# bruAristimunha/Synthetic-Sleep-EEG-Signal-Generation-using-Latent-Diffusion-Models

Hardware: AMD Instinct MI355X
Metric: EEG windows/sec (LDM train step) (higher is better)
Workload: dtype bf16; 1 GPU; LDM train step on raw (B,1,3072) windows: frozen AutoencoderKL[32,32,64] encode+sample x scale, add_noise, config_ldm.yaml UNet (30.5M params, latent_channels=1) fwd+bwd, epsilon MSE, Adam lr 1e-4 [BASELINE configs[2]/[3]: per-GPU batch 256 = global 2048 / 8]; per_gpu_batch=256, global_batch=256, latent_len=768, parallelism=dp1

## Files before the change

include/eegldm.h:

```cpp
#ifndef EEGLDM_H
#define EEGLDM_H
#include <stdint.h>
#ifdef __cplusplus
extern "C" {
#endif

#define EEGLDM_ABI_VERSION 8

enum { EEGLDM_F32 = 0, EEGLDM_BF16 = 1, EEGLDM_F16 = 2 };
enum {
  EEGLDM_OK = 0,
  EEGLDM_ERR_INVALID = -1,
  EEGLDM_ERR_HIP = -2,
  EEGLDM_ERR_UNSUPPORTED = -3,
  EEGLDM_ERR_NOMEM = -4
};
enum { EEGLDM_PRED_EPSILON = 0, EEGLDM_PRED_V = 1, EEGLDM_PRED_SAMPLE = 2 };

typedef struct eegldm_ctx eegldm_ctx;
typedef struct eegldm_unet eegldm_unet;
typedef struct eegldm_aekl eegldm_aekl;
typedef struct eegldm_disc eegldm_disc;
typedef struct eegldm_block eegldm_block;

int eegldm_abi_version(void);
const char* eegldm_last_error(void);
int eegldm_ctx_create(int hip_device, void* hip_stream, int own_stream, eegldm_ctx** out);
void* eegldm_ctx_stream(const eegldm_ctx*);
int eegldm_ctx_destroy(eegldm_ctx* ctx);
int eegldm_ctx_sync(eegldm_ctx* ctx);
int eegldm_timer_start(eegldm_ctx* ctx);
int eegldm_timer_stop_ms(eegldm_ctx* ctx, float* ms_host);
int eegldm_prof_enable(eegldm_ctx* ctx, int on);
int eegldm_prof_summary(eegldm_ctx* ctx, int kernel_class, double* flops_host, double* ms_host, int* launches_host);
int eegldm_prof_bracket_overhead_ms(eegldm_ctx* ctx, double* ms_host);
int eegldm_prof_dump(eegldm_ctx* ctx, const char* path_host);
int eegldm_debug_reload_env(void);
int eegldm_debug_gn_last_route(int backward, int* out6_host);

int eegldm_ncl_to_nlc(eegldm_ctx*, const float* src_ncl, void* dst_nlc, long ld_dst, int B, int C, int L, int dst_dtype);
int eegldm_nlc_to_ncl(eegldm_ctx*, const void* src_nlc, long ld_src, float* dst_ncl, int B, int C, int L, int src_dtype);
int eegldm_pack_conv_weight(eegldm_ctx*, const float* w_ref, float* w_packed, int Cout, int Cin, int K);
int eegldm_unpack_conv_weight(eegldm_ctx*, const float* w_packed, float* w_ref, int Cout, int Cin, int K);
int eegldm_cast(eegldm_ctx*, const float* src, void* dst, long n, int dst_dtype);

int eegldm_conv1d_pack_kblocked(eegldm_ctx*, const void* w, void* w_kblocked, int Cout, int Cin, int dtype);
int eegldm_conv1d_pack_kblocked_k(eegldm_ctx*, const void* w, void* w_kblocked, int Cout, int Cin, int K, int dtype);
int eegldm_conv1d_forget_kblocked(eegldm_ctx*, const void* w);
int eegldm_conv1d_pack_stride2(eegldm_ctx*, const void* w, void* w_fwd, void* w_dgrad, int Cout, int Cin, int dtype);
int eegldm_conv1d_pack_dgrad(eegldm_ctx*, const void* w, void* w_dgrad, int Cout, int Cin, int dtype);
int eegldm_conv1d_pack_dgrad_k(eegldm_ctx*, const void* w, void* w_dgrad, int Cout, int Cin, int K, int dtype);

int eegldm_conv1d_fwd(eegldm_ctx*, const void* x, long ldx, const void* w, const float* bias,
                      void* y, long ldy, int B, int Lin, int Cin, int Cout, int K, int stride,
                      int pad_l, int pad_r, const float* rowvec, long ld_rowvec,
                      const void* resid, long ld_resid, int dtype);
int eegldm_conv1d_skip_fwd(eegldm_ctx*, const void* x, long ldx, const void* w, const float* bias,
                           const void* x2, long ldx2, const void* w2, const float* bias2, void* y, long ldy,
                           int B, int L, int Cin, int Cin2, int Cout, const float* rowvec, long ld_rowvec, int dtype);
int eegldm_conv1d_bwd_data(eegldm_ctx*, const void* dy, long lddy, const void* w, void* dx, long lddx,
                           int B, int Lin, int Cin, int Cout, int K, int stride, int pad_l, int pad_r,
                           const void* resid, long ld_resid, int dtype);
int eegldm_conv1d_bwd_weight(eegldm_ctx*, const void* x, long ldx, const void* dy, long lddy,
                             float* dw, float* dbias, int B, int Lin, int Cin, int Cout, int K,
                             int stride, int pad_l, int pad_r, int dtype);
int eegldm_linear_fwd(eegldm_ctx*, const void* x, long ldx, const void* w, const float* bias, void* y, long ldy,
                      int M, int N, int K, int dtype, int out_f32);
int eegldm_linear_bwd(eegldm_ctx*, const void* x, long ldx, const void* w, const void* dy, long lddy, void* dx, long lddx,
                      float* dw, float* dbias, int M, int N, int K, int dtype, int dx_f32);

int eegldm_groupnorm_fwd(eegldm_ctx*, const void* x, long ldx, const float* gamma, const float* beta,
// ... 274 lines not shown
```

synthetic-sleep-eeg-signal-generation-using-latent-diffusion-models_amd/_lib.py:

```python
import ctypes as C
import os

_HERE = os.path.dirname(os.path.abspath(__file__))
LIB_PATH = os.environ.get("EEGLDM_LIB") or os.path.join(_HERE, "libeegldm.so")

F32, BF16, F16 = 0, 1, 2
PRED = {"epsilon": 0, "v_prediction": 1, "sample": 2}


class LibraryMissing(RuntimeError):
    pass


def _load():
    import torch
    if not os.path.exists(LIB_PATH):
        raise LibraryMissing(f"{LIB_PATH} not found: build it with `make` (python -c 'import __graft_entry__ as g; g.build()')")
    return C.CDLL(LIB_PATH)


lib = _load()
lib.eegldm_last_error.restype = C.c_char_p
if hasattr(lib, "eegldm_ctx_stream"):
    lib.eegldm_ctx_stream.restype = C.c_void_p
if hasattr(lib, 'eegldm_unet_num_params'):
    lib.eegldm_unet_num_params.restype = C.c_long

_vp, _i, _l, _f = C.c_void_p, C.c_int, C.c_long, C.c_float
SIGNATURES = {
    "eegldm_abi_version": [],
    "eegldm_last_error": [],
    "eegldm_ctx_create": [_i, _vp, _i, C.POINTER(_vp)],
    "eegldm_ctx_stream": [_vp],
    "eegldm_ctx_destroy": [_vp],
    "eegldm_ctx_sync": [_vp],
    "eegldm_timer_start": [_vp],
    "eegldm_timer_stop_ms": [_vp, C.POINTER(_f)],
    "eegldm_prof_enable": [_vp, _i],
    "eegldm_prof_summary": [_vp, _i, C.POINTER(C.c_double), C.POINTER(C.c_double), C.POINTER(_i)],
    "eegldm_prof_bracket_overhead_ms": [_vp, C.POINTER(C.c_double)],
    "eegldm_prof_dump": [_vp, C.c_char_p],
    "eegldm_debug_reload_env": [],
    "eegldm_debug_gn_last_route": [_i, _vp],
    "eegldm_ncl_to_nlc": [_vp, _vp, _vp, _l, _i, _i, _i, _i],
    "eegldm_nlc_to_ncl": [_vp, _vp, _l, _vp, _i, _i, _i, _i],
    "eegldm_pack_conv_weight": [_vp, _vp, _vp, _i, _i, _i],
    "eegldm_conv1d_pack_kblocked": [_vp, _vp, _vp, _i, _i, _i],
    "eegldm_conv1d_pack_kblocked_k": [_vp, _vp, _vp, _i, _i, _i, _i],
    "eegldm_batchnorm_lrelu_fwd": [_vp, _vp, _l, _vp, _vp, _vp, _vp, _vp, _vp, _vp, _l, _l, _i, _f, _i, _i],
    "eegldm_batchnorm_lrelu_bwd": [_vp, _vp, _l, _vp, _vp, _vp, _vp, _l, _vp, _l, _vp, _vp, _l, _i, _f, _i],
    "eegldm_kl_reparam_fwd": [_vp, _vp, _vp, _vp, _vp, _vp, _vp, _l, _i, _i],
    "eegldm_kl_reparam_bwd": [_vp, _vp, _vp, _vp, _vp, _vp, _vp, _vp, _l, _f, _i],
    "eegldm_avgpool2_fwd": [_vp, _vp, _l, _vp, _l, _i, _i, _i, _i],
    "eegldm_avgpool2_bwd": [_vp, _vp, _l, _vp, _l, _i, _i, _i, _i],
    "eegldm_nearest2_fwd": [_vp, _vp, _l, _vp, _l, _i, _i, _i, _i],
    "eegldm_nearest2_bwd": [_vp, _vp, _l, _vp, _l, _i, _i, _i, _i],
    "eegldm_conv1d_skip_fwd": [_vp, _vp, _l, _vp, _vp, _vp, _l, _vp, _vp, _vp, _l, _i, _i, _i, _i, _i, _vp, _l, _i],
    "eegldm_comm_unique_id": [_vp],
    "eegldm_comm_create": [_vp, _vp, _i, _i, _vp],
    "eegldm_comm_destroy": [_vp],
    "eegldm_comm_rank": [_vp],
    "eegldm_comm_world": [_vp],
    "eegldm_comm_allreduce_mean_f32": [_vp, _vp, _l, _l],
    "eegldm_comm_broadcast_f32": [_vp, _vp, _l, _i],
    "eegldm_comm_wait": [_vp],
    "eegldm_conv1d_forget_kblocked": [_vp, _vp],
    "eegldm_conv1d_pack_stride2": [_vp, _vp, _vp, _vp, _i, _i, _i],
    "eegldm_conv1d_pack_dgrad": [_vp, _vp, _vp, _i, _i, _i],
    "eegldm_conv1d_pack_dgrad_k": [_vp, _vp, _vp, _i, _i, _i, _i],
    "eegldm_unpack_conv_weight": [_vp, _vp, _vp, _i, _i, _i],
    "eegldm_cast": [_vp, _vp, _vp, _l, _i],
    "eegldm_conv1d_fwd": [_vp, _vp, _l, _vp, _vp, _vp, _l, _i, _i, _i, _i, _i, _i, _i, _i, _vp, _l, _vp, _l, _i],
    "eegldm_conv1d_bwd_data": [_vp, _vp, _l, _vp, _vp, _l, _i, _i, _i, _i, _i, _i, _i, _i, _vp, _l, _i],
    "eegldm_conv1d_bwd_weight": [_vp, _vp, _l, _vp, _l, _vp, _vp, _i, _i, _i, _i, _i, _i, _i, _i, _i],
    "eegldm_linear_fwd": [_vp, _vp, _l, _vp, _vp, _vp, _l, _i, _i, _i, _i, _i],
    "eegldm_linear_bwd": [_vp, _vp, _l, _vp, _vp, _l, _vp, _l, _vp, _vp, _i, _i, _i, _i, _i],
# ... 244 lines not shown
```

synthetic-sleep-eeg-signal-generation-using-latent-diffusion-models_amd/csrc/aekl.hip:

```cpp
#include <stdlib.h>

#include <string>
#include <vector>

#include "aekl_thin.h"
#include "net.h"

int ls_bn_lrelu_fwd(eegldm_ctx*, const void* x, long ldx, const float* gamma, const float* beta, float* stats, float* rmean, float* rvar,
                    float* nbt, void* y, long ldy, long rows, int C, float slope, int training, int dtype);
int ls_bn_lrelu_bwd(eegldm_ctx*, const void* x, long ldx, const float* gamma, const float* beta, const float* stats, const void* dy, long lddy,
                    void* dx, long lddx, float* dgamma, float* dbeta, long rows, int C, float slope, int dtype);
int ls_bn_stats(eegldm_ctx*, const void* x, long ldx, float* stats, float* rmean, float* rvar, float* nbt, long rows, int C, int training, int dtype);
int ls_bn_stats_from_parts(eegldm_ctx*, const float* parts, int nb, float* stats, float* rmean, float* rvar, float* nbt, long rows, int C);
int ls_bn_apply(eegldm_ctx*, const void* x, long ldx, const float* gamma, const float* beta, const float* stats, void* y, long ldy, long rows, int C, float slope, int dtype);
bool disc_tail_ok(int dtype, int C, long ldy);
int disc_tail_fwd(eegldm_ctx*, int dtype, const void* y, long ldy, const float* gamma, const float* beta, const float* stats, const float* w3,
                  const float* bias, float slope, float* logits, int B, int L, int C);
int disc_tail_bwd(eegldm_ctx*, int dtype, const void* y, long ldy, const float* gamma, const float* beta, const float* stats, const float* w3,
                  float slope, const float* dlogits, void* dy, long lddy, float* dgamma, float* dbeta, float* dw3, float* dbias, int B, int L, int C);
bool disc_head_ok(int dtype, int C0, long ldda, int stride, int L, int Lo);
int disc_head_bwd(eegldm_ctx*, int dtype, const void* da, long ldda, const void* x, const void* w, const float* bias, float slope,
                  float* dw, float* db, float* dx, int B, int L, int Lo, int C0, int stride);
int ls_upsample2(eegldm_ctx*, const void* x, long ldx, void* y, long ldy, long rows_in, int C, int dtype);
int ls_upsample2_bwd(eegldm_ctx*, const void* dy, long lddy, void* dx, long lddx, long rows_in, int C, int dtype);
// ... 360 lines not shown
    int ic = oc; oc = nc[i];
    for (int r = 0; r < cfg->num_res_blocks; r++) { dec.push_back(make_res(a, lay, dname(""), ic, oc, G)); bi++; ic = oc; }
    if (i != 0) {
      Op u; u.kind = OP_UPS; dec.push_back(u);
      dec.push_back(make_conv(a, lay, dname(".conv.conv"), ic, ic, 3, 1, 1, 1, true)); bi++;
    }
  }
  dec.push_back(make_gn(a, lay, dname(""), oc, G)); bi++;
  dec.push_back(make_conv(a, lay, dname(".conv"), oc, cfg->out_channels, 3, 1, 1, 1, true)); bi++;
  a->q_mu = make_conv(a, lay, "quant_conv_mu.conv", lat, lat, 1, 1, 0, 0, true);
  a->q_lv = make_conv(a, lay, "quant_conv_log_sigma.conv", lat, lat, 1, 1, 0, 0, true);
  a->dec.push_back(make_conv(a, lay, "post_quant_conv.conv", lat, lat, 1, 1, 0, 0, true));
  for (auto& o : dec) a->dec.push_back(o);
  a->nparams = lay.off;
  *out = a;
  return 0;
}
eegldm_ctx* aekl_ctx(const eegldm_aekl* a) { return a->ctx; }
int aekl_out_channels(const eegldm_aekl* a) { return a->cfg.out_channels; }
int aekl_down(const eegldm_aekl* a) { return 1 << (a->cfg.n_levels - 1); }
extern "C" int eegldm_aekl_destroy(eegldm_aekl* a) { delete a; return 0; }
extern "C" int eegldm_aekl_num_entries(const eegldm_aekl* a) { return (int)a->entries.size(); }
extern "C" long eegldm_aekl_num_params(const eegldm_aekl* a) { return a->nparams; }
extern "C" int eegldm_aekl_entry(const eegldm_aekl* a, int i, char* name, int cap, long* offset, long* numel, int* ndim, int shape[3]) {
  return entry_query(a, i, name, cap, offset, numel, ndim, shape);
}
extern "C" int eegldm_aekl_bind(eegldm_aekl* a, float* params, float* grads) { EEG_CHECK(a && params, "null argument"); return a->bind(params, grads); }
extern "C" int eegldm_aekl_sync_weights(eegldm_aekl* a) { EEG_CHECK(a, "null argument"); return a->sync_weights(); }

namespace {
int lat_len(const eegldm_aekl* a, int L) { return L >> (a->cfg.n_levels - 1); }

bool enc_fused_eligible(const eegldm_aekl* a, int L);
int aekl_encode_fused_seq(eegldm_aekl* a, View x, int B, int& L, View* out);
int aekl_encode_impl(eegldm_aekl* a, const float* x, const float* eps, int B, int L, View* z_out, float* kl, bool frozen = false) {
  EEG_CHECK((L % (1 << (a->cfg.n_levels - 1))) == 0, "L=%d must be divisible by 2^(levels-1)", L);
  eegldm_ctx* ctx = a->ctx; const int dt = a->dtype, lat = a->cfg.latent_channels, cin = a->cfg.in_channels;
  a->arena.reset(); a->rt.clear(); a->tape_enc.clear(); a->tape_dec.clear();
  a->B = B; a->L = L; a->have_tape = false;
  View x0; ALLOC_OR_FAIL(x0.p, a->alloc_act((long)B * L, cin)); x0.ld = cin; x0.C = cin;
  EEG_TRY(eegldm_ncl_to_nlc(ctx, x, x0.p, cin, B, cin, L, dt));
  int Lc = L;
  if (frozen && enc_fused_eligible(a, L)) EEG_TRY(aekl_encode_fused_seq(a, x0, B, Lc, &a->h_enc));
  else EEG_TRY(a->forward_seq(a->enc, x0, B, Lc, &a->h_enc, a->tape_enc, 1));
  a->Ll = Lc;
  const long n = (long)B * Lc * lat;
  ALLOC_OR_FAIL(a->mu.p, a->alloc_act((long)B * Lc, lat)); a->mu.ld = lat; a->mu.C = lat;
  ALLOC_OR_FAIL(a->lv.p, a->alloc_act((long)B * Lc, lat)); a->lv.ld = lat; a->lv.C = lat;
  EEG_TRY(op_conv_fwd(ctx, dt, a->h_enc.p, a->h_enc.ld, a->W(a->q_mu.w), a->P(a->q_mu.b), a->mu.p, lat, B, Lc, lat, lat, 1, 1, 0, 0, nullptr, 0, nullptr, 0));
  EEG_TRY(op_conv_fwd(ctx, dt, a->h_enc.p, a->h_enc.ld, a->W(a->q_lv.w), a->P(a->q_lv.b), a->lv.p, lat, B, Lc, lat, lat, 1, 1, 0, 0, nullptr, 0, nullptr, 0));
  a->eps_nlc = nullptr;
  if (eps) {
    ALLOC_OR_FAIL(a->eps_nlc, a->arena.alloc(sizeof(float) * n));
    EEG_TRY(eegldm_ncl_to_nlc(ctx, eps, a->eps_nlc, lat, B, lat, Lc, EEGLDM_F32));
  }
  ALLOC_OR_FAIL(a->sigma, a->arena.alloc(sizeof(float) * n));
  View z; ALLOC_OR_FAIL(z.p, a->alloc_act((long)B * Lc, lat)); z.ld = lat; z.C = lat;
  if (kl && !ctx->loss_prezeroed) HIP_TRY(hipMemsetAsync(kl, 0, sizeof(float), ctx->stream));
  EEG_TRY(ls_reparam(ctx, a->mu.p, a->lv.p, a->eps_nlc, z.p, a->sigma, kl, n, B, dt));
  *z_out = z;
  return 0;
}
bool enc_fused_eligible(const eegldm_aekl* a, int L) {
  if (getenv("EEGLDM_AEKL_NO_FUSED_ENC") != nullptr) return false;
  if ((a->dtype != EEGLDM_BF16 && a->dtype != EEGLDM_F16) || a->cfg.norm_num_groups != 1) return false;
  int Lc = L; bool any = false;
  for (const Op& o : a->enc) {
    if (o.kind == OP_CONV) Lc = (Lc + o.pl + o.pr - o.k) / o.stride + 1;
    else if (o.kind == OP_RES) { if (!pre_conv3_ok(a->dtype, o.r.cin, o.r.cout, Lc) || !pre_conv3_ok(a->dtype, o.r.cout, o.r.cout, Lc)) return false; any = true; }
    else if (o.kind != OP_GN) return false;
  }
  return any;
}
int aekl_encode_fused_seq(eegldm_aekl* a, View x, int B, int& L, View* out) {
  eegldm_ctx* ctx = a->ctx; const int dt = a->dtype;
  size_t nslots = 0;
  for (const Op& o : a->enc) nslots += (o.kind == OP_RES) ? 2 : 0;
  double* slots; ALLOC_OR_FAIL(slots, (double*)a->arena.alloc(sizeof(double) * 2 * B * (nslots + 1)));
  HIP_TRY(hipMemsetAsync(slots, 0, sizeof(double) * 2 * B * (nslots + 1), ctx->stream));
  size_t used = 0;
  auto next_slot = [&]() { return slots + (used++) * 2 * (size_t)B; };
  double* cur_stats = nullptr;
  for (size_t i = 0; i < a->enc.size(); i++) {
    const Op& o = a->enc[i];
    const bool next_res = i + 1 < a->enc.size() && a->enc[i + 1].kind == OP_RES;
    if (o.kind == OP_CONV) {
      const int Lo = (L + o.pl + o.pr - o.k) / o.stride + 1;
      View y; ALLOC_OR_FAIL(y.p, a->alloc_act((long)B * Lo, o.cout)); y.ld = o.cout; y.C = o.cout;
      EEG_TRY(op_conv_fwd(ctx, dt, x.p, x.ld, a->W(o.w), o.b >= 0 ? a->P(o.b) : nullptr, y.p, y.ld, B, L, o.cin, o.cout, o.k, o.stride, o.pl, o.pr,
                          nullptr, 0, nullptr, 0));
      L = Lo; x = y; cur_stats = nullptr;
      if (next_res) { cur_stats = next_slot(); EEG_TRY(sample_stats_launch(ctx, x.p, (long)L * x.C, B, cur_stats, a->dtype)); }
    } else if (o.kind == OP_RES) {
      const ResDesc& r = o.r;
      EEG_CHECK(cur_stats, "fused encoder: no statistics for a ResBlock input");
      View h1; ALLOC_OR_FAIL(h1.p, a->alloc_act((long)B * L, r.cout)); h1.ld = r.cout; h1.C = r.cout;
      double* st_h1 = next_slot();
      EEG_TRY(pre_conv3_launch(ctx, x.p, cur_stats, a->P(r.gn1_w), a->P(r.gn1_b), a->W(r.c1_w), a->P(r.c1_b), nullptr, h1.p, st_h1, B, L, r.cin, r.cout, GN_EPS, a->dtype));
      View res = x;
      if (r.sk_w >= 0) {
        ALLOC_OR_FAIL(res.p, a->alloc_act((long)B * L, r.cout)); res.ld = r.cout; res.C = r.cout;
        EEG_TRY(op_conv_fwd(ctx, dt, x.p, x.ld, a->W(r.sk_w), a->P(r.sk_b), res.p, res.ld, B, L, r.cin, r.cout, 1, 1, 0, 0, nullptr, 0, nullptr, 0));
      }
      View y; ALLOC_OR_FAIL(y.p, a->alloc_act((long)B * L, r.cout)); y.ld = r.cout; y.C = r.cout;
      double* st_y = next_res ? next_slot() : nullptr;
      EEG_TRY(pre_conv3_launch(ctx, h1.p, st_h1, a->P(r.gn2_w), a->P(r.gn2_b), a->W(r.c2_w), a->P(r.c2_b), res.p, y.p, st_y, B, L, r.cout, r.cout, GN_EPS, a->dtype));
      x = y; cur_stats = st_y;
    } else {
      View y; ALLOC_OR_FAIL(y.p, a->alloc_act((long)B * L, x.C)); y.ld = x.C; y.C = x.C;
      float* st; ALLOC_OR_FAIL(st, (float*)a->arena.alloc(sizeof(float) * 2 * B * o.groups));
      EEG_TRY(eegldm_groupnorm_fwd(ctx, x.p, x.ld, a->P(o.gw), a->P(o.gb), y.p, y.ld, st, B, L, x.C, o.groups, GN_EPS, 0, 0, nullptr, 0, dt));
      x = y; cur_stats = nullptr;
    }
  }
  *out = x;
  return 0;
}

int aekl_export_latents(eegldm_aekl* a, const View& z, float* z_ncl, float* mu_ncl, float* sigma_ncl) {
  const int lat = a->cfg.latent_channels;
  if (z_ncl) EEG_TRY(eegldm_nlc_to_ncl(a->ctx, z.p, lat, z_ncl, a->B, lat, a->Ll, a->dtype));
  if (mu_ncl) EEG_TRY(eegldm_nlc_to_ncl(a->ctx, a->mu.p, lat, mu_ncl, a->B, lat, a->Ll, a->dtype));
  if (sigma_ncl) EEG_TRY(eegldm_nlc_to_ncl(a->ctx, a->sigma, lat, sigma_ncl, a->B, lat, a->Ll, EEGLDM_F32));
  return 0;
}
int aekl_decode_impl(eegldm_aekl* a, const View& z, int B, int Ll, float* recon) {
  int Lc = Ll; View y;
  EEG_TRY(a->forward_seq(a->dec, z, B, Lc, &y, a->tape_dec, 1));
  return eegldm_nlc_to_ncl(a->ctx, y.p, y.ld, recon, B, a->cfg.out_channels, Lc, a->dtype);
}
}

extern "C" int eegldm_aekl_encode(eegldm_aekl* a, const float* x, const float* eps, float* z, float* z_mu, float* z_sigma, int B, int L) {
  EEG_CHECK(a && x && a->params, "null argument / unbound parameters");
  View zv;
  EEG_TRY(aekl_encode_impl(a, x, eps, B, L, &zv, nullptr, true));
  return aekl_export_latents(a, zv, z, z_mu, z_sigma);
}
extern "C" int eegldm_aekl_decode(eegldm_aekl* a, const float* z, float* recon, int B, int Ll) {
  EEG_CHECK(a && z && recon && a->params, "null argument / unbound parameters");
  const int lat = a->cfg.latent_channels;
  a->arena.reset(); a->rt.clear(); a->tape_enc.clear(); a->tape_dec.clear(); a->have_tape = false;
  View zv; ALLOC_OR_FAIL(zv.p, a->alloc_act((long)B * Ll, lat)); zv.ld = lat; zv.C = lat;
  EEG_TRY(eegldm_ncl_to_nlc(a->ctx, z, zv.p, lat, B, lat, Ll, a->dtype));
  return aekl_decode_impl(a, zv, B, Ll, recon);
}
extern "C" int eegldm_aekl_forward(eegldm_aekl* a, const float* x, const float* eps, float* recon, float* z_mu, float* z_sigma, float* kl, int B, int L) {
  EEG_CHECK(a && x && recon && a->params, "null argument / unbound parameters");
  a->thin_tape = false;
  if (thin_ready(a, L)) {
    ThinProgram& p = a->thin;
    a->arena.reset(); a->rt.clear(); a->tape_enc.clear(); a->tape_dec.clear(); a->have_tape = false;
    a->B = B; a->L = L; a->Ll = p.Ll;
    ALLOC_OR_FAIL(p.tape, a->arena.alloc(sizeof(float) * (size_t)B * p.tape_stride));
    ALLOC_OR_FAIL(p.stats, a->arena.alloc(sizeof(float) * (size_t)B * p.nstat * 2));
    a->thin_eps = nullptr;
    if (eps) {
      ALLOC_OR_FAIL(a->thin_eps, a->arena.alloc(sizeof(float) * (size_t)B * p.lat * p.Ll));
      HIP_TRY(hipMemcpyAsync(a->thin_eps, eps, sizeof(float) * (size_t)B * p.lat * p.Ll, hipMemcpyDeviceToDevice, a->ctx->stream));
    }
    if (kl && !a->ctx->loss_prezeroed) HIP_TRY(hipMemsetAsync(kl, 0, sizeof(float), a->ctx->stream));
    EEG_TRY(thin_forward(a->ctx, p, a->params, x, a->thin_eps, recon, z_mu, z_sigma, kl, B));
    a->have_tape = true; a->thin_tape = true;
    return 0;
  }
  View zv;
  EEG_TRY(aekl_encode_impl(a, x, eps, B, L, &zv, kl));
  EEG_TRY(aekl_export_latents(a, zv, nullptr, z_mu, z_sigma));
  EEG_TRY(aekl_decode_impl(a, zv, B, a->Ll, recon));
  a->have_tape = true;
// ... 246 lines not shown
```

synthetic-sleep-eeg-signal-generation-using-latent-diffusion-models_amd/csrc/internal.h:

```cpp
#pragma once
#include "common.h"

int ew_temb(eegldm_ctx*, const int64_t* t, void* out, int B, int dim, int dtype);
int ew_silu(eegldm_ctx*, const float* x, void* y, long n, int dtype);
int ew_silu_bwd(eegldm_ctx*, const float* dy, const float* x, void* dx, long n, int dtype);
int eeg_det_buffer(eegldm_ctx*, size_t bytes, float** out);
int ew_fold_partials_det(eegldm_ctx*, const float* parts, int nparts, long stride, int off, int n, float* total);
int ew_colsum(eegldm_ctx*, const void* x, long ldx, float* out_ps, long ldo, float* total, int B, int L, int C, int dtype);
int ew_softmax(eegldm_ctx*, const float* S, void* P, long rows, int n, int dtype);
int ew_softmax_bwd(eegldm_ctx*, const float* dP, const void* P, void* dS, long rows, int n, float alpha, int dtype);
int ew_add_rows(eegldm_ctx*, void* dst, long ldd, const void* src, long lds, long rows, int C, int dtype);
int ew_dropout_rows(eegldm_ctx*, void* x, long ld, long rows, int C, float p, uint64_t seed, uint64_t offset, int dtype);
int ew_film_silu_fwd(eegldm_ctx*, const void* hn, long ldh, const float* emb, long lde, void* a, long lda, int B, int L, int C, int dtype);
int ew_film_silu_bwd(eegldm_ctx*, const void* hn, long ldh, const float* emb, long lde, const void* da, long ldda, void* dhn, long lddh,
                     float* demb, long ldde, int B, int L, int C, int dtype);
int ew_copy_rows(eegldm_ctx*, void* dst, long ldd, const void* src, long lds, long rows, int C, int dtype);
int ew_label_emb_add(eegldm_ctx*, float* emb, long ld, const int64_t* y, const float* table, int B, int te, int K);
int ew_label_emb_grad(eegldm_ctx*, const float* demb, long ld, const int64_t* y, int B, int te, int K, float* dtable);
int ew_label_dropout(eegldm_ctx*, const int64_t* y, int64_t* out, int B, float p, int64_t null_class, uint64_t seed, uint64_t offset);
int ew_emb_gather(eegldm_ctx*, const float* table, const int64_t* y, int K, int w, float* out, int B);

bool conv_is_thin(int Cin, int Cout, int dtype);
struct KbDesc { long off; long chunk0; int cout, cin; };
int kblk_pack(eegldm_ctx* ctx, const void* w_plain, void* w_packed, const KbDesc* d_table, int n, long total_chunks);
// ... 29 lines not shown
                const float* rowvec, long ld_rowvec, const void* resid, long ldr, float act_slope = 0.f,
                float* col_parts = nullptr, int* col_nparts = nullptr);
bool op_conv_fuses_act(int dtype, int Cin, int Cout, int K, long ldy);
int op_conv3_skip_fwd(eegldm_ctx*, int dtype, const void* x, long ldx, const void* w, const float* bias, const void* x2, long ldx2,
                      const void* w2, const float* bias2, void* y, long ldy, int B, int L, int Cin, int Cin2, int Cout,
                      const float* rowvec, long ld_rowvec);
int op_conv_dgrad(eegldm_ctx*, int dtype, const void* dy, long lddy, const void* w, void* dx, long lddx,
                  int B, int Lin, int Cin, int Cout, int K, int stride, int pad_l, int pad_r, const void* resid, long ldr);
bool op_wgrad_fuses_bias(int dtype, int Cin, int Cout);
int op_gn_fold_flush(eegldm_ctx*);
int op_wgrad_flush(eegldm_ctx*);
int op_conv_wgrad(eegldm_ctx*, int dtype, const void* x, long ldx, const void* dy, long lddy, float* dw, float* dbias,
                  int B, int Lin, int Cin, int Cout, int K, int stride, int pad_l, int pad_r);
int op_linear(eegldm_ctx*, int dtype, const void* x, long ldx, const void* w, long ldw, const float* bias, void* y, long ldy,
              int M, int N, int K, int out_f32);
int op_linear_dgrad(eegldm_ctx*, int dtype, const void* dy, long lddy, const void* w, long ldw, void* dx, long lddx,
                    int M, int N, int K, int out_f32);
int op_linear_wgrad(eegldm_ctx*, int dtype, const void* x, long ldx, const void* dy, long lddy, float* dw, long lddw,
                    int M, int N, int K);
int op_attention_fwd(eegldm_ctx*, int dtype, const void* qkv, long ldq, void* out, long ldo, void* probs, float* logits,
                     int B, int T, int C);
int op_attention_bwd(eegldm_ctx*, int dtype, const void* qkv, long ldq, const void* probs, const void* dout, long lddo,
                     void* dqkv, long lddq, float* dprobs, void* dlogits, int B, int T, int C);
int op_groupnorm_bwd(eegldm_ctx*, const void* x, long ldx, const float* gamma, const float* beta, const float* stats,
                     const void* dy, long lddy, void* dx, long lddx, float* dgamma, float* dbeta, int B, int L, int C, int G,
                     int fuse_silu, int resample, const void* dxr, long lddxr, int dtype, float* colsum_ps, long ldps, int* colsum_done,
                     const void* dxr2 = nullptr, long lddxr2 = 0, int* dxr2_done = nullptr, int* slots_deferred = nullptr, int defer_region = 0);
int op_gn_slot_reduce_deferred(eegldm_ctx*, float* dgamma, float* dbeta, int C, int region = 0);
int ew_fold_partials(eegldm_ctx*, const float* parts, int nparts, int n, float* total);
bool pre_conv3_ok(int dtype, int Cin, int Cout, int L);
int pre_conv3_launch(eegldm_ctx*, const void* x, const double* in_stats, const float* gamma, const float* beta, const void* w,
                     const float* bias, const void* resid, void* y, double* out_stats, int B, int L, int Cin, int Cout, float eps, int dtype);
int sample_stats_launch(eegldm_ctx*, const void* x, long n_per_sample, int B, double* stats, int dtype);
bool attn_chain_ok(int dtype, int T, int C, long ldq, long ldo);
int attn_chain_fwd(eegldm_ctx*, const void* qkv, long ldq, void* out, long ldo, void* probs, int B, int T, int C, int dtype);
int attn_chain_bwd(eegldm_ctx*, const void* qkv, long ldq, const void* probs, const void* dout, long lddo, void* dq, long lddq,
                   void* dS, int B, int T, int C, int fuse_kv, int dtype);
bool attn_chain_bwd_fuses_kv(eegldm_ctx*, int B, int T);
```

Before: 14170 windows/s.

## Fuse frozen encoder tail into one per-window persistent kernel

Adds a single-kernel encoder path that keeps the post-downsample activations of one window in registers and LDS. It runs the downsample convs, ResBlocks, GroupNorm, the output conv, the mu/logvar projections and the reparameterisation in one block per sample, writing NCL latents directly. This removes many kernel launches and the global-memory round trips between encoder layers, plus the separate latent export. The cost is one 1024-thread block per sample with large LDS, which limits occupancy, and a very specialised code path that needs shape checks and has an env var to disable it.

Result: no change. 14310 windows/s, median of 6 (+1.0%).

```diff
diff --git a/include/eegldm.h b/include/eegldm.h
--- a/include/eegldm.h
+++ b/include/eegldm.h
@@ -37,6 +37,7 @@
 int eegldm_prof_dump(eegldm_ctx* ctx, const char* path_host);
 int eegldm_debug_reload_env(void);
 int eegldm_debug_gn_last_route(int backward, int* out6_host);
+int eegldm_debug_aekl_last_encode_route(int* out_host);
 
 int eegldm_ncl_to_nlc(eegldm_ctx*, const float* src_ncl, void* dst_nlc, long ld_dst, int B, int C, int L, int dst_dtype);
 int eegldm_nlc_to_ncl(eegldm_ctx*, const void* src_nlc, long ld_src, float* dst_ncl, int B, int C, int L, int src_dtype);
diff --git a/synthetic-sleep-eeg-signal-generation-using-latent-diffusion-models_amd/_lib.py b/synthetic-sleep-eeg-signal-generation-using-latent-diffusion-models_amd/_lib.py
--- a/synthetic-sleep-eeg-signal-generation-using-latent-diffusion-models_amd/_lib.py
+++ b/synthetic-sleep-eeg-signal-generation-using-latent-diffusion-models_amd/_lib.py
@@ -42,6 +42,7 @@
     "eegldm_prof_dump": [_vp, C.c_char_p],
     "eegldm_debug_reload_env": [],
     "eegldm_debug_gn_last_route": [_i, _vp],
+    "eegldm_debug_aekl_last_encode_route": [_vp],
     "eegldm_ncl_to_nlc": [_vp, _vp, _vp, _l, _i, _i, _i, _i],
     "eegldm_nlc_to_ncl": [_vp, _vp, _l, _vp, _i, _i, _i, _i],
     "eegldm_pack_conv_weight": [_vp, _vp, _vp, _i, _i, _i],
diff --git a/synthetic-sleep-eeg-signal-generation-using-latent-diffusion-models_amd/csrc/aekl.hip b/synthetic-sleep-eeg-signal-generation-using-latent-diffusion-models_amd/csrc/aekl.hip
--- a/synthetic-sleep-eeg-signal-generation-using-latent-diffusion-models_amd/csrc/aekl.hip
+++ b/synthetic-sleep-eeg-signal-generation-using-latent-diffusion-models_amd/csrc/aekl.hip
@@ -416,8 +416,14 @@
 int lat_len(const eegldm_aekl* a, int L) { return L >> (a->cfg.n_levels - 1); }
 
 bool enc_fused_eligible(const eegldm_aekl* a, int L);
-int aekl_encode_fused_seq(eegldm_aekl* a, View x, int B, int& L, View* out);
-int aekl_encode_impl(eegldm_aekl* a, const float* x, const float* eps, int B, int L, View* z_out, float* kl, bool frozen = false) {
+int aekl_encode_fused_seq(eegldm_aekl* a, View x, int B, int& L, View* out, size_t end);
+struct EncWindowPlan { size_t split; int C0, C1, C2; };
+bool enc_window_eligible(const eegldm_aekl* a, int L, EncWindowPlan* plan);
+int aekl_encode_window(eegldm_aekl* a, const EncWindowPlan& plan, View x0, const float* eps, int B, int L, float* z, float* mu, float* sigma);
+enum { ENC_ROUTE_LAYERS = 0, ENC_ROUTE_FUSED = 1, ENC_ROUTE_WINDOW = 2 };
+thread_local int g_enc_last_route = -1;
+struct EncNcl { float *z, *mu, *sigma; bool exported; };
+int aekl_encode_impl(eegldm_aekl* a, const float* x, const float* eps, int B, int L, View* z_out, float* kl, bool frozen = false, EncNcl* ncl = nullptr) {
   EEG_CHECK((L % (1 << (a->cfg.n_levels - 1))) == 0, "L=%d must be divisible by 2^(levels-1)", L);
   eegldm_ctx* ctx = a->ctx; const int dt = a->dtype, lat = a->cfg.latent_channels, cin = a->cfg.in_channels;
   a->arena.reset(); a->rt.clear(); a->tape_enc.clear(); a->tape_dec.clear();
@@ -425,8 +431,19 @@
   View x0; ALLOC_OR_FAIL(x0.p, a->alloc_act((long)B * L, cin)); x0.ld = cin; x0.C = cin;
   EEG_TRY(eegldm_ncl_to_nlc(ctx, x, x0.p, cin, B, cin, L, dt));
   int Lc = L;
-  if (frozen && enc_fused_eligible(a, L)) EEG_TRY(aekl_encode_fused_seq(a, x0, B, Lc, &a->h_enc));
-  else EEG_TRY(a->forward_seq(a->enc, x0, B, Lc, &a->h_enc, a->tape_enc, 1));
+  EncWindowPlan plan;
+  if (frozen && ncl && !kl && enc_window_eligible(a, L, &plan)) {
+    EEG_TRY(aekl_encode_window(a, plan, x0, eps, B, L, ncl->z, ncl->mu, ncl->sigma));
+    a->Ll = lat_len(a, L); ncl->exported = true; g_enc_last_route = ENC_ROUTE_WINDOW;
+    return 0;
+  }
+  if (frozen && enc_fused_eligible(a, L)) {
+    EEG_TRY(aekl_encode_fused_seq(a, x0, B, Lc, &a->h_enc, a->enc.size()));
+    g_enc_last_route = ENC_ROUTE_FUSED;
+  } else {
+    EEG_TRY(a->forward_seq(a->enc, x0, B, Lc, &a->h_enc, a->tape_enc, 1));
+    if (frozen) g_enc_last_route = ENC_ROUTE_LAYERS;
+  }
   a->Ll = Lc;
   const long n = (long)B * Lc * lat;
   ALLOC_OR_FAIL(a->mu.p, a->alloc_act((long)B * Lc, lat)); a->mu.ld = lat; a->mu.C = lat;
@@ -456,7 +473,48 @@
   }
   return any;
 }
-int aekl_encode_fused_seq(eegldm_aekl* a, View x, int B, int& L, View* out) {
+bool enc_window_eligible(const eegldm_aekl* a, int L, EncWindowPlan* plan) {
+  if (getenv("EEGLDM_AEKL_NO_WINDOW_ENC") != nullptr || !enc_fused_eligible(a, L)) return false;
+  const eegldm_aekl_cfg& c = a->cfg;
+  if (c.num_res_blocks != 2 || (c.n_levels != 2 && c.n_levels != 3) || c.in_channels != 1 || c.latent_channels != 1) return false;
+  const int* nc = c.num_channels;
+  for (int i = 0; i < c.n_levels; i++) {
+    if ((nc[i] != 32 && nc[i] != 64) || (L >> i) % 256 != 0 || (L >> i) << i != L) return false;
+  }
+  const size_t nops = 1 + 3 * (size_t)c.n_levels - 1 + 2;
+  if (a->enc.size() != nops) return false;
+  const Op& dn = a->enc[3];
+  if (dn.kind != OP_CONV || dn.stride != 2 || dn.k != 3 || dn.pl != 0 || dn.pr != 1) return false;
+  plan->split = 3; plan->C0 = nc[0]; plan->C1 = nc[1]; plan->C2 = c.n_levels == 3 ? nc[2] : 0;
+  return enc_window_ok(a->dtype, plan->C0, plan->C1, plan->C2, L);
+}
+int aekl_encode_window(eegldm_aekl* a, const EncWindowPlan& plan, View x0, const float* eps, int B, int L, float* z, float* mu, float* sigma) {
+  int Lc = L; View h0;
+  EEG_TRY(aekl_encode_fused_seq(a, x0, B, Lc, &h0, plan.split));
+  EEG_CHECK(Lc == L && h0.C == plan.C0 && h0.ld == plan.C0, "window encoder: unexpected level-0 tensor");
+  EncWindowArgs w = {};
+  w.x = (const bf16_t*)h0.p; w.L0 = L; w.wT = (const bf16_t*)a->wT; w.P = a->params;
+  size_t i = plan.split;
+  const int nlev = plan.C2 != 0 ? 2 : 1;
+  for (int lv = 0; lv < nlev; lv++) {
+    const Op& dn = a->enc[i++];
+    EEG_CHECK(dn.kind == OP_CONV && dn.stride == 2 && dn.b >= 0, "window encoder: expected a stride-2 conv");
+    w.dn_w[lv] = dn.w; w.dn_b[lv] = dn.b;
+    for (int r = 0; r < 2; r++) {
+      const Op& o = a->enc[i++];
+      EEG_CHECK(o.kind == OP_RES, "window encoder: expected a ResBlock");
+      const ResDesc& d = o.r;
+      w.res[2 * lv + r] = EncWindowRes{d.gn1_w, d.gn1_b, d.c1_w, d.c1_b, d.gn2_w, d.gn2_b, d.c2_w, d.c2_b, d.sk_w, d.sk_b};
+    }
+  }
+  const Op& gn = a->enc[i++]; const Op& co = a->enc[i++];
+  EEG_CHECK(gn.kind == OP_GN && co.kind == OP_CONV && co.cout == 1 && co.k == 3 && co.stride == 1 && co.b >= 0 && i == a->enc.size(), "window encoder: unexpected tail");
+  w.gn_w = gn.gw; w.gn_b = gn.gb; w.co_w = co.w; w.co_b = co.b;
+  w.mu_w = a->q_mu.w; w.mu_b = a->q_mu.b; w.lv_w = a->q_lv.w; w.lv_b = a->q_lv.b;
+  w.noise = eps; w.z = z; w.mu = mu; w.sigma = sigma; w.eps = GN_EPS;
+  return enc_window_launch(a->ctx, w, B, plan.C0, plan.C1, plan.C2, a->dtype);
+}
+int aekl_encode_fused_seq(eegldm_aekl* a, View x, int B, int& L, View* out, size_t end) {
   eegldm_ctx* ctx = a->ctx; const int dt = a->dtype;
   size_t nslots = 0;
   for (const Op& o : a->enc) nslots += (o.kind == OP_RES) ? 2 : 0;
@@ -465,7 +523,7 @@
   size_t used = 0;
   auto next_slot = [&]() { return slots + (used++) * 2 * (size_t)B; };
   double* cur_stats = nullptr;
-  for (size_t i = 0; i < a->enc.size(); i++) {
+  for (size_t i = 0; i < end; i++) {
     const Op& o = a->enc[i];
     const bool next_res = i + 1 < a->enc.size() && a->enc[i + 1].kind == OP_RES;
     if (o.kind == OP_CONV) {
@@ -517,9 +575,15 @@
 
 extern "C" int eegldm_aekl_encode(eegldm_aekl* a, const float* x, const float* eps, float* z, float* z_mu, float* z_sigma, int B, int L) {
   EEG_CHECK(a && x && a->params, "null argument / unbound parameters");
-  View zv;
-  EEG_TRY(aekl_encode_impl(a, x, eps, B, L, &zv, nullptr, true));
+  View zv; EncNcl ncl = {z, z_mu, z_sigma, false};
+  EEG_TRY(aekl_encode_impl(a, x, eps, B, L, &zv, nullptr, true, &ncl));
+  if (ncl.exported) return 0;
   return aekl_export_latents(a, zv, z, z_mu, z_sigma);
+}
+extern "C" int eegldm_debug_aekl_last_encode_route(int* out_host) {
+  EEG_CHECK(out_host, "null argument");
+  *out_host = g_enc_last_route;
+  return 0;
 }
 extern "C" int eegldm_aekl_decode(eegldm_aekl* a, const float* z, float* recon, int B, int Ll) {
   EEG_CHECK(a && z && recon && a->params, "null argument / unbound parameters");
diff --git a/synthetic-sleep-eeg-signal-generation-using-latent-diffusion-models_amd/csrc/enc_window.hip b/synthetic-sleep-eeg-signal-generation-using-latent-diffusion-models_amd/csrc/enc_window.hip
--- /dev/null
+++ b/synthetic-sleep-eeg-signal-generation-using-latent-diffusion-models_amd/csrc/enc_window.hip
@@ -0,0 +1,297 @@
+#include "common.h"
+#include "internal.h"
+
+namespace {
+
+constexpr int WT = 256;
+constexpr int WTHREADS = 1024;
+constexpr int WRED = 256;
+
+template <typename T16>
+__device__ __forceinline__ void mma16w(const uint4& a, const uint4& b, f32x4& acc) {
+  if constexpr (Is16<T16>::f16) acc = __builtin_amdgcn_mfma_f32_16x16x32_f16(__builtin_bit_cast(f16x8, a), __builtin_bit_cast(f16x8, b), acc, 0, 0, 0);
+  else acc = __builtin_amdgcn_mfma_f32_16x16x32_bf16(__builtin_bit_cast(bf16x8, a), __builtin_bit_cast(bf16x8, b), acc, 0, 0, 0);
+}
+template <typename T16> __device__ __forceinline__ float round16(float v) { return w16_lo<T16>(pack16x2<T16>(v, 0.f)); }
+
+struct Lane { int tid, lane, lm, q, wv; };
+
+__device__ __forceinline__ void keep_packed(uint2& v) { asm volatile("" : "+v"(v.x), "+v"(v.y)); }
+
+template <int CTRL> __device__ __forceinline__ float dpp_add(float v) {
+  return v + __builtin_bit_cast(float, __builtin_amdgcn_update_dpp(0, __builtin_bit_cast(int, v), CTRL, 0xF, 0xF, true));
+}
+__device__ __forceinline__ float quad_sum(float v) { return dpp_add<0x4E>(dpp_add<0xB1>(v)); }
+__device__ __forceinline__ float wave_sum_dpp(float v) {
+  v = dpp_add<0x140>(dpp_add<0x141>(quad_sum(v)));
+  const int i = __builtin_bit_cast(int, v);
+  return ((__builtin_bit_cast(float, __builtin_amdgcn_readlane(i, 0)) + __builtin_bit_cast(float, __builtin_amdgcn_readlane(i, 16))) +
+          __builtin_bit_cast(float, __builtin_amdgcn_readlane(i, 32))) + __builtin_bit_cast(float, __builtin_amdgcn_readlane(i, 48));
+}
+
+enum { ST_ACT = 0, ST_NORM = 1, ST_RAW = 2 };
+template <typename T16, int C, int MODE, bool RAW2>
+__device__ __forceinline__ void win_stage(char* A, char* A2, const uint2 (&cur)[12], int ntiles, float mean, float rstd,
+                                          const float* __restrict__ gamma, const float* __restrict__ beta, const Lane& ln) {
+  constexpr int PA = C * 2 + 16, NF = C / 16, MAXT = 12 / NF;
+  float sc[NF][4], sh[NF][4];
+  if constexpr (MODE != ST_RAW) {
+#pragma unroll
+    for (int f = 0; f < NF; f++) {
+      const float4 g = *(const float4*)(gamma + f * 16 + ln.q * 4), bt = *(const float4*)(beta + f * 16 + ln.q * 4);
+      sc[f][0] = g.x * rstd; sc[f][1] = g.y * rstd; sc[f][2] = g.z * rstd; sc[f][3] = g.w * rstd;
+      sh[f][0] = bt.x - mean * sc[f][0]; sh[f][1] = bt.y - mean * sc[f][1]; sh[f][2] = bt.z - mean * sc[f][2]; sh[f][3] = bt.w - mean * sc[f][3];
+    }
+  }
+  __syncthreads();
+#pragma unroll
+  for (int t = 0; t < MAXT; t++) {
+    if (t < ntiles) {
+      const int off = (t * WT + ln.wv * 16 + ln.lm + 1) * PA + ln.q * 8;
+#pragma unroll
+      for (int f = 0; f < NF; f++) {
+        uint2 v = cur[t * NF + f];
+        keep_packed(v);
+        uint2 o = v;
+        if constexpr (MODE != ST_RAW) {
+          float u0 = fmaf(w16_lo<T16>(v.x), sc[f][0], sh[f][0]), u1 = fmaf(w16_hi<T16>(v.x), sc[f][1], sh[f][1]);
+          float u2 = fmaf(w16_lo<T16>(v.y), sc[f][2], sh[f][2]), u3 = fmaf(w16_hi<T16>(v.y), sc[f][3], sh[f][3]);
+          if constexpr (MODE == ST_ACT) { u0 = silu_f(u0); u1 = silu_f(u1); u2 = silu_f(u2); u3 = silu_f(u3); }
+          o.x = pack16x2<T16>(u0, u1); o.y = pack16x2<T16>(u2, u3);
+        }
+        *(uint2*)(A + off + f * 32) = o;
+        if constexpr (RAW2) *(uint2*)(A2 + off + f * 32) = v;
+      }
+    }
+  }
+  if (ln.tid < PA / 8) {
+    const int last = (ntiles * WT + 1) * PA;
+    *(uint2*)(A + ln.tid * 8) = make_uint2(0u, 0u); *(uint2*)(A + last + ln.tid * 8) = make_uint2(0u, 0u);
+    if constexpr (RAW2) { *(uint2*)(A2 + ln.tid * 8) = make_uint2(0u, 0u); *(uint2*)(A2 + last + ln.tid * 8) = make_uint2(0u, 0u); }
+  }
+  __syncthreads();
+}
+
+template <typename T16, int CI, int CO, int STRIDE, int TAPS, bool RESID, bool STATS>
+__device__ __forceinline__ void win_conv(const char* a0, int tstride, const bf16_t* __restrict__ w, const float* __restrict__ bias, int t0, int t1,
+                                         const uint2 (&res)[12], uint2 (&out)[12], float& s1, float& s2, const Lane& ln) {
+  constexpr int PA = CI * 2 + 16, KS = CI / 32, NF = CO / 16, MAXT = 12 / NF, NJ = CI == 64 ? 1 : 2, NH = NF / NJ;
+  const int lane_off = ln.lm * CI + ln.q * 8;
+#pragma unroll
+  for (int h = 0; h < NH; h++) {
+    uint4 wf[TAPS][KS][NJ];
+#pragma unroll
+    for (int t = 0; t < TAPS; t++)
+#pragma unroll
+      for (int ks = 0; ks < KS; ks++)
+#pragma unroll
+        for (int j = 0; j < NJ; j++) {
+          const bf16_t* wu = w + (t * CO + (h * NJ + j) * 16) * CI + ks * 32;
+          wf[t][ks][j] = *(const uint4*)(wu + lane_off);
+        }
+    float4 bv[NJ];
+#pragma unroll
+    for (int j = 0; j < NJ; j++) bv[j] = *(const float4*)(bias + (h * NJ + j) * 16 + ln.q * 4);
+#pragma unroll
+    for (int t = 0; t < MAXT; t++) {
+      if (t >= t0 && t < t1) {
+        const char* ar = a0 + (tstride * t + STRIDE * (ln.wv * 16 + ln.lm)) * PA + ln.q * 16;
+        f32x4 acc[NJ];
+#pragma unroll
+        for (int j = 0; j < NJ; j++) acc[j] = f32x4{0.f, 0.f, 0.f, 0.f};
+#pragma unroll
+        for (int tap = 0; tap < TAPS; tap++) {
+#pragma unroll
+          for (int ks = 0; ks < KS; ks++) {
+            const uint4 af = *(const uint4*)(ar + tap * PA + ks * 64);
+#pragma unroll
+            for (int j = 0; j < NJ; j++) mma16w<T16>(wf[tap][ks][j], af, acc[j]);
+          }
+          if constexpr (CI == 64) __builtin_amdgcn_sched_barrier(0);
+        }
+#pragma unroll
+        for (int j = 0; j < NJ; j++) {
+          const int f = h * NJ + j;
+          float v[4] = {acc[j][0] + bv[j].x, acc[j][1] + bv[j].y, acc[j][2] + bv[j].z, acc[j][3] + bv[j].w};
+          if constexpr (RESID) {
+            uint2 rr = res[t * NF + f];
+            keep_packed(rr);
+            v[0] += w16_lo<T16>(rr.x); v[1] += w16_hi<T16>(rr.x); v[2] += w16_lo<T16>(rr.y); v[3] += w16_hi<T16>(rr.y);
+          }
+          uint2 o; o.x = pack16x2<T16>(v[0], v[1]); o.y = pack16x2<T16>(v[2], v[3]);
+          if constexpr (STATS) {
+            const float r0 = w16_lo<T16>(o.x), r1 = w16_hi<T16>(o.x), r2 = w16_lo<T16>(o.y), r3 = w16_hi<T16>(o.y);
+            s1 += (r0 + r1) + (r2 + r3);
+            s2 += fmaf(r0, r0, r1 * r1) + fmaf(r2, r2, r3 * r3);
+          }
+          keep_packed(o);
+          out[t * NF + f] = o;
+        }
+        __builtin_amdgcn_sched_barrier(0);
+      }
+    }
+  }
+}
+
+__device__ __forceinline__ void win_stats(float s1, float s2, double* red, double n, float eps, float& mean, float& rstd, const Lane& ln) {
+  s1 = wave_sum_dpp(s1); s2 = wave_sum_dpp(s2);
+  if (ln.lane == 0) { red[2 * ln.wv] = (double)s1; red[2 * ln.wv + 1] = (double)s2; }
+  __syncthreads();
+  double a = 0.0, b = 0.0;
+#pragma unroll
+  for (int i = 0; i < WTHREADS / 64; i++) { a += red[2 * i]; b += red[2 * i + 1]; }
+  const double m = a / n;
+  double var = b / n - m * m; if (var < 0.0) var = 0.0;
+  mean = (float)m; rstd = (float)(1.0 / sqrt(var + (double)eps));
+}
+
+template <typename T16, int CI, int CO, bool STATS_OUT>
+__device__ __forceinline__ void win_res(const EncWindowArgs& a, const EncWindowRes& r, char* A, double* red, uint2 (&cur)[12], uint2 (&res)[12],
+                                        int ntiles, float& mean, float& rstd, const Lane& ln) {
+  const int L = ntiles * WT;
+  char* A2 = A + (L + 2) * (CI * 2 + 16);
+  float s1 = 0.f, s2 = 0.f, d1 = 0.f, d2 = 0.f;
+  win_stage<T16, CI, ST_ACT, CI != CO>(A, A2, cur, ntiles, mean, rstd, a.P + r.gn1_w, a.P + r.gn1_b, ln);
+  if constexpr (CI == CO) {
+#pragma unroll
+    for (int i = 0; i < 12; i++) { res[i] = cur[i]; keep_packed(res[i]); }
+  } else {
+    win_conv<T16, CI, CO, 1, 1, false, false>(A2 + (CI * 2 + 16), WT, a.wT + r.sk_w, a.P + r.sk_b, 0, ntiles, res, res, d1, d2, ln);
+  }
+  win_conv<T16, CI, CO, 1, 3, false, true>(A, WT, a.wT + r.c1_w, a.P + r.c1_b, 0, ntiles, cur, cur, s1, s2, ln);
+  win_stats(s1, s2, red, (double)CO * (double)L, a.eps, mean, rstd, ln);
+  win_stage<T16, CO, ST_ACT, false>(A, A, cur, ntiles, mean, rstd, a.P + r.gn2_w, a.P + r.gn2_b, ln);
+  s1 = s2 = 0.f;
+  win_conv<T16, CO, CO, 1, 3, true, STATS_OUT>(A, WT, a.wT + r.c2_w, a.P + r.c2_b, 0, ntiles, res, cur, s1, s2, ln);
+  if constexpr (STATS_OUT) win_stats(s1, s2, red, (double)CO * (double)L, a.eps, mean, rstd, ln);
+}
+
+template <typename T16, int C0, int C1, int C2>
+__global__ __launch_bounds__(WTHREADS) void enc_window_kernel(const EncWindowArgs a) {
+  extern __shared__ __attribute__((aligned(16))) char sm[];
+  double* red = (double*)sm;
+  char* A = sm + WRED;
+  Lane ln; ln.tid = threadIdx.x; ln.lane = ln.tid & 63; ln.lm = ln.lane & 15; ln.q = ln.lane >> 4; ln.wv = ln.tid >> 6;
+  const int b = blockIdx.x;
+  uint2 cur[12], res[12];
+#pragma unroll
+  for (int i = 0; i < 12; i++) cur[i] = res[i] = make_uint2(0u, 0u);
+  float mean = 0.f, rstd = 0.f, s1 = 0.f, s2 = 0.f;
+  int L = a.L0 / 2, ntiles = L / WT;
+  {
+    constexpr int PA = C0 * 2 + 16, SEGS = C0 / 8;
+    const bf16_t* xs = a.x + (long)b * a.L0 * C0;
+#pragma unroll 1
+    for (int p = 0; p < ntiles; p++) {
+      __syncthreads();
+      for (int c = ln.tid; c < (2 * WT + 1) * SEGS; c += WTHREADS) {
+        const int r = c / SEGS, sg = c - r * SEGS, pos = 2 * WT * p + r;
+        *(uint4*)(A + r * PA + sg * 16) = pos < a.L0 ? *(const uint4*)(xs + (long)pos * C0 + sg * 8) : make_uint4(0u, 0u, 0u, 0u);
+      }
+      __syncthreads();
+      win_conv<T16, C0, C0, 2, 3, false, true>(A, 0, a.wT + a.dn_w[0], a.P + a.dn_b[0], p, p + 1, cur, cur, s1, s2, ln);
+    }
+  }
+  win_stats(s1, s2, red, (double)C0 * (double)L, a.eps, mean, rstd, ln);
+  win_res<T16, C0, C1, true>(a, a.res[0], A, red, cur, res, ntiles, mean, rstd, ln);
+  win_res<T16, C1, C1, C2 == 0>(a, a.res[1], A, red, cur, res, ntiles, mean, rstd, ln);
+  constexpr int CL = C2 != 0 ? C2 : C1;
+  if constexpr (C2 != 0) {
+    win_stage<T16, C1, ST_RAW, false>(A, A, cur, ntiles, 0.f, 0.f, nullptr, nullptr, ln);
+    L /= 2; ntiles = L / WT;
+    s1 = s2 = 0.f;
+    win_conv<T16, C1, C1, 2, 3, false, true>(A + (C1 * 2 + 16), 2 * WT, a.wT + a.dn_w[1], a.P + a.dn_b[1], 0, ntiles, cur, cur, s1, s2, ln);
+    win_stats(s1, s2, red, (double)C1 * (double)L, a.eps, mean, rstd, ln);
+    win_res<T16, C1, C2, true>(a, a.res[2], A, red, cur, res, ntiles, mean, rstd, ln);
+    win_res<T16, C2, C2, true>(a, a.res[3], A, red, cur, res, ntiles, mean, rstd, ln);
+  }
+  win_stage<T16, CL, ST_NORM, false>(A, A, cur, ntiles, mean, rstd, a.P + a.gn_w, a.P + a.gn_b, ln);
+  {
+    constexpr int PA = CL * 2 + 16, CPT = CL / 4;
+    const int part = ln.tid & 3;
+    float wo[3][CPT];
+#pragma unroll
+    for (int t = 0; t < 3; t++)
+#pragma unroll
+      for (int e = 0; e < CPT; e += 2) {
+        const unsigned u = *(const unsigned*)(a.wT + a.co_w + t * CL + part * CPT + e);
+        wo[t][e] = w16_lo<T16>(u); wo[t][e + 1] = w16_hi<T16>(u);
+      }
+    const float b_out = a.P[a.co_b];
+    const float w_mu = ld_f32((const T16*)a.wT + a.mu_w), b_mu = a.P[a.mu_b], w_lv = ld_f32((const T16*)a.wT + a.lv_w), b_lv = a.P[a.lv_b];
+    for (int l = ln.tid >> 2; l < L; l += WTHREADS / 4) {
+      float acc = 0.f;
+#pragma unroll
+      for (int t = 0; t < 3; t++) {
+        const char* row = A + (l + t) * PA + part * CPT * 2;
+#pragma unroll
+        for (int e = 0; e < CPT; e += 8) {
+          const uint4 v = *(const uint4*)(row + e * 2);
+          const unsigned in[4] = {v.x, v.y, v.z, v.w};
+#pragma unroll
+          for (int k = 0; k < 4; k++) { acc = fmaf(w16_lo<T16>(in[k]), wo[t][e + 2 * k], acc); acc = fmaf(w16_hi<T16>(in[k]), wo[t][e + 2 * k + 1], acc); }
+        }
+      }
+      acc = quad_sum(acc);
+      if (part == 0) {
+        const float hv = round16<T16>(acc + b_out);
+        const float mu = round16<T16>(fmaf(hv, w_mu, b_mu));
+        float lv = round16<T16>(fmaf(hv, w_lv, b_lv));
+        lv = lv < -30.0f ? -30.0f : (lv > 20.0f ? 20.0f : lv);
+        const float sg = expf(0.5f * lv);
+        const long o = (long)b * L + l;
+        if (a.z) a.z[o] = a.noise ? round16<T16>(mu + a.noise[o] * sg) : mu;
+        if (a.mu) a.mu[o] = mu;
+        if (a.sigma) a.sigma[o] = sg;
+      }
+    }
+  }
+}
+
+int lds_row_bytes(int C) { return C * 2 + 16; }
+
+}
+
+static int win_max_rows(int C) { return C == 32 ? 6 * WT : 3 * WT; }
+
+bool enc_window_ok(int dtype, int C0, int C1, int C2, int L0) {
+  if (dtype != EEGLDM_BF16 && dtype != EEGLDM_F16) return false;
+  if ((C0 != 32 && C0 != 64) || (C1 != 32 && C1 != 64) || (C2 != 0 && C2 != 32 && C2 != 64)) return false;
+  if (C1 < C0 || (C2 != 0 && C2 < C1)) return false;
+  const int L1 = L0 / 2, L2 = L0 / 4;
+  if (L0 <= 0 || L0 % 2 != 0 || L1 % WT != 0 || L1 > win_max_rows(C1) || L1 > win_max_rows(C0)) return false;
+  if (C2 != 0 && (L1 % 2 != 0 || L2 % WT != 0 || L2 > win_max_rows(C2))) return false;
+  return true;
+}
+
+int enc_window_launch(eegldm_ctx* ctx, const EncWindowArgs& args, int B, int C0, int C1, int C2, int dtype) {
+  EEG_CHECK(enc_window_ok(dtype, C0, C1, C2, args.L0), "enc_window: unsupported encoder %d / %d / %d at L %d", C0, C1, C2, args.L0);
+  const int L1 = args.L0 / 2, L2 = L1 / 2;
+  long need = (long)(2 * WT + 1) * lds_row_bytes(C0);
+  auto level = [&](int Cin, int C, int L) {
+    const long a = (long)(L + 2) * lds_row_bytes(Cin) * (Cin != C ? 2 : 1), c = (long)(L + 2) * lds_row_bytes(C);
+    if (a > need) need = a;
+    if (c > need) need = c;
+  };
+  level(C0, C1, L1);
+  if (C2 != 0) level(C1, C2, L2);
+  const int lds = (int)need + WRED;
+  EEG_CHECK(lds <= 160 * 1024, "enc_window: %d bytes of LDS", lds);
+#define ENCW_T(c0, c1, c2, T) do {                                                                                                   \
+    static DevOnce attr;                                                                                                              \
+    if (attr.need(ctx->device)) HIP_TRY(hipFuncSetAttribute((const void*)enc_window_kernel<T, c0, c1, c2>, hipFuncAttributeMaxDynamicSharedMemorySize, 160 * 1024)); \
+    hipLaunchKernelGGL((enc_window_kernel<T, c0, c1, c2>), dim3(B), dim3(WTHREADS), lds, ctx->stream, args);                         \
+  } while (0)
+#define ENCW(c0, c1, c2) do { if (dtype == EEGLDM_F16) ENCW_T(c0, c1, c2, f16_t); else ENCW_T(c0, c1, c2, bf16_t); } while (0)
+  if (C0 == 32 && C1 == 32 && C2 == 64) ENCW(32, 32, 64);
+  else if (C0 == 32 && C1 == 64 && C2 == 0) ENCW(32, 64, 0);
+  else if (C0 == 32 && C1 == 32 && C2 == 0) ENCW(32, 32, 0);
+  else if (C0 == 32 && C1 == 32 && C2 == 32) ENCW(32, 32, 32);
+  else if (C0 == 32 && C1 == 64 && C2 == 64) ENCW(32, 64, 64);
+  else if (C0 == 64 && C1 == 64 && C2 == 0) ENCW(64, 64, 0);
+  else ENCW(64, 64, 64);
+#undef ENCW
+#undef ENCW_T
+  LAUNCH_CHECK();
+  return 0;
+}
diff --git a/synthetic-sleep-eeg-signal-generation-using-latent-diffusion-models_amd/csrc/internal.h b/synthetic-sleep-eeg-signal-generation-using-latent-diffusion-models_amd/csrc/internal.h
--- a/synthetic-sleep-eeg-signal-generation-using-latent-diffusion-models_amd/csrc/internal.h
+++ b/synthetic-sleep-eeg-signal-generation-using-latent-diffusion-models_amd/csrc/internal.h
@@ -85,6 +85,19 @@
 int pre_conv3_launch(eegldm_ctx*, const void* x, const double* in_stats, const float* gamma, const float* beta, const void* w,
                      const float* bias, const void* resid, void* y, double* out_stats, int B, int L, int Cin, int Cout, float eps, int dtype);
 int sample_stats_launch(eegldm_ctx*, const void* x, long n_per_sample, int B, double* stats, int dtype);
+struct EncWindowRes { long gn1_w, gn1_b, c1_w, c1_b, gn2_w, gn2_b, c2_w, c2_b, sk_w, sk_b; };
+struct EncWindowArgs {
+  const bf16_t* x; int L0;
+  const bf16_t* wT; const float* P;
+  long dn_w[2], dn_b[2];
+  EncWindowRes res[4];
+  long gn_w, gn_b, co_w, co_b, mu_w, mu_b, lv_w, lv_b;
+  const float* noise;
+  float *z, *mu, *sigma;
+  float eps;
+};
+bool enc_window_ok(int dtype, int C0, int C1, int C2, int L0);
+int enc_window_launch(eegldm_ctx*, const EncWindowArgs&, int B, int C0, int C1, int C2, int dtype);
 bool attn_chain_ok(int dtype, int T, int C, long ldq, long ldo);
 int attn_chain_fwd(eegldm_ctx*, const void* qkv, long ldq, void* out, long ldo, void* probs, int B, int T, int C, int dtype);
 int attn_chain_bwd(eegldm_ctx*, const void* qkv, long ldq, const void* probs, const void* dout, long lddo, void* dq, long lddq,
```
